# jim-berend/semanticlens

Hardware: AMD Instinct MI355X
Metric: images/sec concept-db build (higher is better)
Workload: dtype f32 (encoder GEMMs split-bf16x3, fp32 accumulate)

## Files before the change

include/semanticlens_amd.h:

```cpp
#ifndef SEMANTICLENS_AMD_H
#define SEMANTICLENS_AMD_H

#include <stddef.h>
#include <stdint.h>

#ifdef __cplusplus
extern "C" {
#endif

#define SL_ABI_VERSION 1

#define SL_E_INVALID (-1)
#define SL_E_HIP (-2)
#define SL_E_UNSUPPORTED (-3)

#define SL_F32 0
#define SL_F16 1
#define SL_BF16 2

#define SL_CONV_MAX 0
#define SL_CONV_MEAN 1
#define SL_CONV_SUM 2

#define SL_TOK_MEAN 0
// ... 126 lines not shown
                        uint16_t* d_out_split, void* stream);
int sl_attention_pool(const float* d_q, const float* d_kv, int64_t kv_row_stride, int64_t v_offset, int64_t B, int64_t T,
                      int64_t H, int64_t head_dim, float* d_out, void* stream);
int sl_patchify(const float* d_img, int64_t B, int64_t C, int64_t Hi, int64_t Wi, int64_t P, float* d_out,
                uint16_t* d_out_split, void* stream);
int sl_attention_pool_q(const float* d_q, int64_t q_batch_stride, const float* d_kv, int64_t kv_row_stride, int64_t v_offset,
                        int64_t B, int64_t T, int64_t H, int64_t head_dim, float* d_out, void* stream);
int sl_tokens_from_map(const float* d_map, int64_t B, int64_t C, int64_t S, const float* d_pos, float* d_out, void* stream);
int sl_broadcast_row(const float* d_v, const float* d_add, int64_t G, int64_t group_stride_elems, int64_t N, float* d_out,
                     void* stream);
int sl_embed_tokens(const float* d_table, int64_t vocab, const int64_t* d_ids, int64_t B, int64_t T, int64_t W,
                    const float* d_pos, float* d_out, void* stream);

#define SL_PP_SHORTEST 0
#define SL_PP_SQUASH 1
#define SL_PP_BICUBIC 0
#define SL_PP_BILINEAR 1
#define SL_PP_PLAN_STRIDE 16
#define SL_PP_INFO_WS_BYTES 0
#define SL_PP_INFO_COEF_BYTES 1
#define SL_PP_INFO_MAX_H 2
#define SL_PP_INFO_PIXEL_BYTES 3
int sl_preprocess_plan(const int32_t* h_hw, const int64_t* h_pixel_offsets, int64_t B, int S, int resize_mode,
                       int interp, int64_t* h_plan, int64_t* h_info);
int sl_preprocess(const uint8_t* d_pixels, const int64_t* d_plan, int64_t B, int S, int interp, int64_t max_h,
                  int64_t coef_bytes, const float* h_mean, const float* h_std, float* d_out, uint8_t* d_out_u8,
                  void* d_ws, size_t ws_bytes, void* stream);
int sl_preprocess_plan_rois(const int32_t* h_hw, const int64_t* h_pixel_offsets, int64_t N, const int64_t* h_index,
                            const int32_t* h_box, int64_t P, int S, int resize_mode, int interp, int64_t* h_plan,
                            int64_t* h_info);

#define SL_RENDER_CROP 0
#define SL_RENDER_OPAQUE 1
#define SL_RENDER_LIGHTEN 2
size_t sl_render_ws_bytes(int64_t B, int64_t H, int64_t W);
int sl_render_heatmaps(const float* d_rel, int64_t B, int64_t Cin, int64_t H, int64_t W, const float* d_img, int kernel_size,
                       float vis_th, float crop_th, double alpha, int style, int rf, float* d_heat, int32_t* d_box,
                       int32_t* d_flags, uint8_t* d_rgb, void* d_ws, size_t ws_bytes, void* stream);
int sl_condition_init(const float* d_act, int64_t B, int64_t C, int64_t S, int64_t sb, int64_t sc, int64_t ss,
                      const int64_t* d_channels, int rf, float* d_out, int64_t ob, int64_t oc, int64_t os, void* stream);

int sl_activation_heat_boxes(const float* d_act, int64_t B, int64_t C, int64_t S, int64_t sb, int64_t sc, int64_t ss,
                             int64_t prefix, int64_t gh, int64_t gw, const int64_t* d_rows, const int64_t* d_channels,
                             int64_t P, int64_t H, int64_t W, int kernel_size, float crop_th, float* d_heat, int32_t* d_box,
                             void* d_ws, size_t ws_bytes, void* stream);
int sl_heat_boxes(const float* d_heat, int64_t P, int64_t H, int64_t W, int kernel_size, float crop_th, int32_t* d_box,
                  void* d_ws, size_t ws_bytes, void* stream);

int sl_batchnorm_infer(const float* d_x, int64_t B, int64_t C, int64_t HW, const float* d_mean, const float* d_var,
                       const float* d_scale, const float* d_bias, double eps, int relu, float* d_y, void* stream);
int sl_batchnorm_infer_add_relu(const float* d_x, const float* d_residual, int64_t B, int64_t C, int64_t HW,
                                const float* d_mean, const float* d_var, const float* d_scale, const float* d_bias,
                                double eps, float* d_y, void* stream);

int sl_topk_init(float* d_vals, int64_t* d_ids, int64_t R, int64_t k, void* stream);
int sl_topk_merge(float* d_vals, int64_t* d_ids, int64_t R, int64_t k, const float* d_cand, int64_t ld, int64_t B,
                  int64_t id_base, void* d_ws, size_t ws_bytes, void* stream);
size_t sl_topk_merge_ws_bytes(int64_t R, int64_t k, int64_t B);
int sl_topk_merge_states(float* d_vals, int64_t* d_ids, int64_t R, int64_t k, const float* d_other_vals,
                         const int64_t* d_other_ids, int64_t M, void* stream);

int sl_cosine_nt(const float* d_x, int64_t M, const float* d_y, int64_t N, int64_t K, float* d_out, void* d_ws,
                 size_t ws_bytes, void* stream);
size_t sl_cosine_nt_ws_bytes(int64_t M, int64_t N, int64_t K);

#define SL_PROF_REDUCE 0
#define SL_PROF_MERGE 1
#define SL_PROF_GEMM 2
#define SL_PROF_GATHER 3
#define SL_PROF_SCORES 4
#define SL_PROF_BATCHNORM 5
#define SL_PROF_TOPK 6
#define SL_PROF_NFAM 7
int sl_prof_enable(int on);
int sl_prof_reset(void);
int sl_prof_read(int family, double* total_ms, int64_t* launches, double* work);

#ifdef __cplusplus
}
#endif
#endif
```

semanticlens_amd/_native.py:

```python
from __future__ import annotations

import ctypes
import operator
import os
from pathlib import Path

import torch

_PKG = Path(__file__).resolve().parent
LIB_PATH = _PKG / "lib" / "libsemanticlens_hip.so"

SL_F32, SL_F16, SL_BF16 = 0, 1, 2
SL_CONV_MAX, SL_CONV_MEAN, SL_CONV_SUM = 0, 1, 2
SL_TOK_MEAN, SL_TOK_ABSMEAN, SL_TOK_MAX, SL_TOK_ABSMAX, SL_TOK_TOKEN = 0, 1, 2, 3, 4
SL_TIES_TOTAL, SL_TIES_ATEN = 0, 1
SL_MAX_SLOTS = 16
SL_PROF_REDUCE, SL_PROF_MERGE, SL_PROF_GEMM, SL_PROF_GATHER, SL_PROF_SCORES, SL_PROF_BATCHNORM, SL_PROF_TOPK = 0, 1, 2, 3, 4, 5, 6
SL_ACT_NONE, SL_ACT_GELU, SL_ACT_QUICKGELU, SL_ACT_GELU_TANH = 0, 1, 2, 3
TIE_MODES = {"total": SL_TIES_TOTAL, "aten": SL_TIES_ATEN}
SL_PP_PLAN_STRIDE = 16
PP_RESIZE_MODES = {"shortest": 0, "squash": 1}
PP_INTERP = {"bicubic": 0, "bilinear": 1}
SL_RENDER_CROP, SL_RENDER_OPAQUE, SL_RENDER_LIGHTEN = 0, 1, 2
RENDER_STYLES = {"crop": SL_RENDER_CROP, "opaque": SL_RENDER_OPAQUE, "lighten": SL_RENDER_LIGHTEN}
# ... 28 lines not shown
    "sl_comm_destroy": (_int, [_vp]),
    "sl_comm_info": (_int, [_vp, ctypes.POINTER(_int), ctypes.POINTER(_int), ctypes.POINTER(_int)]),
    "sl_comm_allgather": (_int, [_vp, _vp, _vp, _i64, _vp]),
    "sl_comm_allreduce": (_int, [_vp, _vp, _i64, _int, _int, _vp]),
    "sl_actmax_packed_bytes": (_sz, [_int, _vp, _i64]),
    "sl_actmax_pack": (_int, [_int, _vp, _vp, _vp, _i64, _vp, _vp]),
    "sl_actmax_merge_packed": (_int, [_int, _vp, _vp, _vp, _i64, _vp, _i64, _i64, _vp]),
    "sl_actmax_allgather_merge_ws_bytes": (_sz, [_int, _vp, _i64, _int]),
    "sl_actmax_allgather_merge": (_int, [_vp, _int, _vp, _vp, _vp, _i64, _vp, _sz, _vp]),
    "sl_gather_rows": (_int, [_vp, _i64, _i64, _vp, _i64, _vp, _vp, _vp]),
    "sl_gather_rows_shard": (_int, [_vp, _i64, _i64, _vp, _i64, _i64, _i64, _vp, _vp, _vp]),
    "sl_similarity": (_int, [_vp, _i64, _i64, _vp, _i64, _i64, _vp, _vp, _sz, _vp]),
    "sl_similarity_ws_bytes": (_sz, [_i64, _i64, _i64, _i64]),
    "sl_set_gemm_mode": (_int, [_int]),
    "sl_set_reduce_policy": (_int, [_i64, _i64]),
    "sl_abs_norm_rows": (_int, [_vp, _i64, _i64, ctypes.c_float, _vp]),
    "sl_similarity_multi": (_int, [_vp, _i64, _i64, _vp, _vp, _int, _vp, _vp, _sz, _vp]),
    "sl_similarity_multi_ws_bytes": (_sz, [_i64, _i64, _vp, _int]),
    "sl_clarity": (_int, [_vp, _i64, _i64, _i64, _vp, _vp]),
    "sl_clarity_multi": (_int, [_vp, _vp, _int, _i64, _i64, _vp, _vp]),
    "sl_redundancy": (_int, [_vp, _i64, _i64, _i64, _vp, _vp, _sz, _vp]),
    "sl_redundancy_ws_bytes": (_sz, [_i64, _i64, _i64]),
    "sl_template_mean": (_int, [_vp, _vp, _i64, _i64, _i64, _vp, _vp]),
    "sl_poly2means": (_int, [_vp, _i64, _i64, _i64, _vp, _int, _vp, _int, _vp, _vp, _vp, _sz, _vp]),
    "sl_poly2means_ws_bytes": (_sz, [_i64, _i64, _i64]),
    "sl_kmeans_trials": (_int, [_int]),
    "sl_polykmeans": (_int, [_vp, _i64, _i64, _i64, _int, _vp, _int, _vp, _int, _vp, _vp, _vp, _sz, _vp]),
    "sl_polykmeans_ws_bytes": (_sz, [_i64, _i64, _i64, _int, _int]),
    "sl_linear": (_int, [_vp, _i64, _i64, _vp, _i64, _vp, _int, _vp, _vp, _i64, _i64, _i64, _i64, _vp, _vp]),
    "sl_layernorm": (_int, [_vp, _i64, _i64, _i64, _vp, _vp, ctypes.c_float, _vp, _vp, _i64, _vp]),
    "sl_attention": (_int, [_vp, _i64, _i64, _i64, _i64, _int, _vp, _vp, _vp]),
    "sl_attention_bf16x3": (_int, [_vp, _i64, _i64, _i64, _i64, _int, _vp, _vp, _vp]),
    "sl_patchify": (_int, [_vp, _i64, _i64, _i64, _i64, _i64, _vp, _vp, _vp]),
    "sl_attention_pool": (_int, [_vp, _vp, _i64, _i64, _i64, _i64, _i64, _i64, _vp, _vp]),
    "sl_attention_pool_q": (_int, [_vp, _i64, _vp, _i64, _i64, _i64, _i64, _i64, _i64, _vp, _vp]),
    "sl_tokens_from_map": (_int, [_vp, _i64, _i64, _i64, _vp, _vp, _vp]),
    "sl_split_elems": (_sz, [_i64, _i64]),
    "sl_split_bf16": (_int, [_vp, _vp, _i64, _i64, _vp, _vp]),
    "sl_linear_bf16x3": (_int, [_vp, _i64, _i64, _vp, _i64, _vp, _int, _vp, _vp, _vp, _i64, _i64, _i64, _i64, _vp, _vp]),
    "sl_broadcast_row": (_int, [_vp, _vp, _i64, _i64, _i64, _vp, _vp]),
    "sl_embed_tokens": (_int, [_vp, _i64, _vp, _i64, _i64, _i64, _vp, _vp, _vp]),
    "sl_preprocess_plan": (_int, [_vp, _vp, _i64, _int, _int, _int, _vp, _vp]),
    "sl_preprocess": (_int, [_vp, _vp, _i64, _int, _int, _i64, _i64, _vp, _vp, _vp, _vp, _vp, _sz, _vp]),
    "sl_render_ws_bytes": (_sz, [_i64, _i64, _i64]),
    "sl_render_heatmaps": (_int, [_vp, _i64, _i64, _i64, _i64, _vp, _int, ctypes.c_float, ctypes.c_float, ctypes.c_double, _int, _int,
                                  _vp, _vp, _vp, _vp, _vp, _sz, _vp]),
    "sl_condition_init": (_int, [_vp, _i64, _i64, _i64, _i64, _i64, _i64, _vp, _int, _vp, _i64, _i64, _i64, _vp]),
    "sl_preprocess_plan_rois": (_int, [_vp, _vp, _i64, _vp, _vp, _i64, _int, _int, _int, _vp, _vp]),
    "sl_activation_heat_boxes": (_int, [_vp, _i64, _i64, _i64, _i64, _i64, _i64, _i64, _i64, _i64, _vp, _vp, _i64, _i64, _i64, _int,
                                        ctypes.c_float, _vp, _vp, _vp, _sz, _vp]),
    "sl_heat_boxes": (_int, [_vp, _i64, _i64, _i64, _int, ctypes.c_float, _vp, _vp, _sz, _vp]),
    "sl_batchnorm_infer": (_int, [_vp, _i64, _i64, _i64, _vp, _vp, _vp, _vp, ctypes.c_double, _int, _vp, _vp]),
    "sl_batchnorm_infer_add_relu": (_int, [_vp, _vp, _i64, _i64, _i64, _vp, _vp, _vp, _vp, ctypes.c_double, _vp, _vp]),
    "sl_topk_init": (_int, [_vp, _vp, _i64, _i64, _vp]),
    "sl_topk_merge": (_int, [_vp, _vp, _i64, _i64, _vp, _i64, _i64, _i64, _vp, _sz, _vp]),
    "sl_topk_merge_ws_bytes": (_sz, [_i64, _i64, _i64]),
    "sl_topk_merge_states": (_int, [_vp, _vp, _i64, _i64, _vp, _vp, _i64, _vp]),
    "sl_cosine_nt": (_int, [_vp, _i64, _vp, _i64, _i64, _vp, _vp, _sz, _vp]),
    "sl_cosine_nt_ws_bytes": (_sz, [_i64, _i64, _i64]),
    "sl_prof_enable": (_int, [_int]),
    "sl_prof_reset": (_int, []),
    "sl_prof_read": (_int, [_int, ctypes.POINTER(ctypes.c_double), ctypes.POINTER(_i64), ctypes.POINTER(ctypes.c_double)]),
}

_lib = None


class NativeLibraryError(RuntimeError):
    """The HIP library is missing or a native call failed."""


def lib():
    global _lib
    if _lib is None:
        path = Path(os.environ.get("SEMANTICLENS_AMD_LIB", LIB_PATH))
        if not path.exists():
            raise NativeLibraryError(
                f"{path} not found. semanticlens_amd has no CPU fallback: build the HIP library first "
                "(python -c 'import __graft_entry__ as g; g.build()' or make -C semanticlens_amd/csrc)."
            )
        handle = ctypes.CDLL(str(path))
        for name, (res, args) in SIGNATURES.items():
            fn = getattr(handle, name)
            fn.restype = res
            fn.argtypes = args
        _lib = handle
    return _lib


def _check(rc: int, what: str) -> int:
    if rc < 0:
        msg = lib().sl_last_error().decode("utf-8", "replace")
        if rc == -1:
            raise ValueError(msg or f"{what}: invalid argument")
        raise NativeLibraryError(f"{what} failed ({rc}): {msg}")
    return rc


def default_device() -> torch.device:
    if not torch.cuda.is_available():
        raise NativeLibraryError(
            "semanticlens_amd needs a HIP device (MI355X): torch.cuda.is_available() is False and there is "
            "no CPU fallback for the concept-DB hot path."
        )
    return torch.device("cuda", torch.cuda.current_device())

# ... 623 lines not shown
    with _on(x.device):
        rc = lib().sl_cosine_nt(_ptr(x), M, _ptr(y), Nn, K, _ptr(out), _ptr(ws), ws.numel(), _stream(x))
    _check(rc, "sl_cosine_nt")
    return out


def topk_chunk_rows(R: int, n_cols: int, tile_bytes: int = TOPK_TILE_BYTES) -> int:
    return max(1, min(n_cols, tile_bytes // (4 * max(R, 1))))


def topk_probe(x: torch.Tensor, y: torch.Tensor, k: int, chunk_rows: int | None = None, id_base: int = 0, state=None):
    k = check_topk_k(k)
    if x.ndim != 2 or y.ndim != 2:
        raise ValueError("topk_probe expects 2-D tensors")
    if y.shape[1] != x.shape[1]:
        raise ValueError(f"embedding widths differ: {x.shape[1]} vs {y.shape[1]}")
    if chunk_rows is not None and chunk_rows < 1:
        raise ValueError(f"chunk_rows = {chunk_rows} must be at least 1")
    xd = _f32c(x)
    yd = _f32c(y, xd.device)
    R, n = xd.shape[0], yd.shape[0]
    vals, ids = state if state is not None else topk_new(R, k, xd.device)
    if R == 0 or n == 0:
        return vals, ids
    step = min(chunk_rows or topk_chunk_rows(R, n), n)
    tile = torch.empty(R * step, dtype=torch.float32, device=xd.device)
    ws = torch.empty(int(lib().sl_cosine_nt_ws_bytes(R, step, xd.shape[1])), dtype=torch.uint8, device=xd.device)
    merge_bytes = int(lib().sl_topk_merge_ws_bytes(R, k, step))
    merge_ws = torch.empty(merge_bytes, dtype=torch.uint8, device=xd.device) if merge_bytes else None
    for start in range(0, n, step):
        rows = min(step, n - start)
        out = tile[: R * rows].view(R, rows)
        cosine_nt(xd, yd[start : start + rows], out, ws)
        topk_merge(vals, ids, out, id_base + start, merge_ws)
    return vals, ids


BN_MAX_CHANNELS = 4096
BN_MAX_ELEMENTS = (1 << 31) - 1


def batchnorm_infer(x: torch.Tensor, mean: torch.Tensor, var: torch.Tensor, weight: torch.Tensor, bias: torch.Tensor, eps: float,
                    relu: bool = False, residual: torch.Tensor | None = None) -> torch.Tensor:
    B, C, H, W = x.shape
    out = torch.empty_like(x)
    with _on(x.device):
        if residual is None:
            rc = lib().sl_batchnorm_infer(_ptr(x), B, C, H * W, _ptr(mean), _ptr(var), _ptr(weight), _ptr(bias), float(eps),
                                          1 if relu else 0, _ptr(out), _stream(x))
        else:
            rc = lib().sl_batchnorm_infer_add_relu(_ptr(x), _ptr(residual), B, C, H * W, _ptr(mean), _ptr(var), _ptr(weight),
                                                   _ptr(bias), float(eps), _ptr(out), _stream(x))
    _check(rc, "sl_batchnorm_infer")
    return out


def prof_enable(on: bool = True):
    _check(lib().sl_prof_enable(1 if on else 0), "sl_prof_enable")


def prof_reset():
    _check(lib().sl_prof_reset(), "sl_prof_reset")


def prof_read(family: int):
    ms, n, w = ctypes.c_double(), _i64(), ctypes.c_double()
    _check(lib().sl_prof_read(family, ctypes.byref(ms), ctypes.byref(n), ctypes.byref(w)), "sl_prof_read")
    return ms.value, n.value, w.value


POLY2_MAX_N = 128


POLYK_MAX_N = 1024
POLYK_MAX_CLUSTERS = 16
POLYK_MAX_COMPONENTS = 65535


def _poly_ws_budget() -> int:
    import os

    return int(float(os.environ.get("SL_POLY_WS_GB", "8")) * (1 << 30))


def poly2means(V: torch.Tensor, first_center, rand, replace_empty_clusters: bool = True, n_clusters: int = 2) -> torch.Tensor:
    import numpy as np

    Vd = _f32c(V)
    if Vd.ndim != 3:
        raise ValueError("polysemanticity_score expects a (n_components, n_samples, n_features) tensor")
    C, n, D = Vd.shape
    first_center = np.ascontiguousarray(first_center, dtype=np.int32)
    rand = np.ascontiguousarray(rand, dtype=np.float64)
    n_init = int(first_center.shape[0])
    out = torch.empty((C,), dtype=torch.float64, device=Vd.device)
    mincnt = torch.empty((C,), dtype=torch.int32, device=Vd.device)
    general = n_clusters != 2 or n > POLY2_MAX_N
    if general:
        if n_clusters > POLYK_MAX_CLUSTERS:
            raise ValueError(f"n_clusters={n_clusters} exceeds the device kernel's maximum of {POLYK_MAX_CLUSTERS}")
        if n > POLYK_MAX_N:
            raise ValueError(f"n_samples={n} exceeds the device kernel's maximum of {POLYK_MAX_N} samples per component")
    if C == 0:
        return out
    per_comp = int(lib().sl_polykmeans_ws_bytes(1, n, D, n_clusters, n_init)) if general else int(lib().sl_poly2means_ws_bytes(1, n, D))
    chunk = max(1, min(C, POLYK_MAX_COMPONENTS, _poly_ws_budget() // max(per_comp, 1)))
# ... 385 lines not shown
```

semanticlens_amd/component_visualization/_bn_fuse.py:

```python
from __future__ import annotations

import inspect
import operator
import os
import warnings
import weakref

import torch
import torch.nn as nn
import torch.nn.functional as F

from .. import _native as N

_BN_FORWARD = nn.modules.batchnorm._BatchNorm.forward
_PLANS: "weakref.WeakKeyDictionary[nn.Module, _Plan]" = weakref.WeakKeyDictionary()
_ADDS = (operator.add, operator.iadd, torch.add)
_RELUS = (F.relu, torch.relu, torch.relu_)


def enabled() -> bool:
    return os.environ.get("SEMANTICLENS_AMD_FUSE_BN", "1") != "0"


def _plain_bn(m) -> bool:
    return isinstance(m, nn.BatchNorm2d) and type(m).forward is _BN_FORWARD


def _plain_relu(m) -> bool:
    return isinstance(m, nn.ReLU) and type(m).forward is nn.ReLU.forward


def _hooked(m: nn.Module) -> bool:
    mod = nn.modules.module
    return bool(m._forward_hooks or m._forward_pre_hooks or mod._global_forward_hooks or mod._global_forward_pre_hooks)


def _streamable(t) -> bool:
    return (isinstance(t, torch.Tensor) and t.is_cuda and t.dtype is torch.float32 and t.dim() == 4 and not t.requires_grad
            and t.is_contiguous() and not t.is_contiguous(memory_format=torch.channels_last) and t.data_ptr() % 16 == 0)


class _Site:

    __slots__ = ("bn", "verified", "dropped")

    def __init__(self, bn: nn.BatchNorm2d):
        self.bn = bn
        self.verified: set = set()
        self.dropped = False

    def eligible(self, x) -> bool:
        bn = self.bn
        if self.dropped or bn.training or torch.is_grad_enabled() or not enabled():
            return False
        if not _streamable(x) or not 0 < x.numel() <= N.BN_MAX_ELEMENTS or x.shape[1] > N.BN_MAX_CHANNELS:
            return False
        if not torch.backends.cudnn.enabled or torch.is_autocast_enabled():
            return False
        for p in (bn.running_mean, bn.running_var, bn.weight, bn.bias):
            if p is None or p.dtype is not torch.float32 or p.device != x.device or not p.is_contiguous() or p.numel() != x.shape[1]:
                return False
        return True

    def run(self, x, relu: bool, other=None, bn_first: bool = True):
        bn = self.bn
        out = N.batchnorm_infer(x, bn.running_mean, bn.running_var, bn.weight, bn.bias, bn.eps, relu=relu, residual=other)
        key = (relu, other is not None, (x.shape[2] * x.shape[3]) % 4 == 0)
        if key in self.verified:
            return out
        ref = F.batch_norm(x, bn.running_mean, bn.running_var, bn.weight, bn.bias, False, 0.0, bn.eps)
        if other is not None:
            ref = ref + other if bn_first else other + ref
        if relu:
            ref = torch.relu_(ref)
        if torch.equal(out.view(torch.int32), ref.view(torch.int32)):
            self.verified.add(key)
            return out
        self.dropped = True
        warnings.warn(
            f"the fused BatchNorm kernel did not reproduce PyTorch's result bit for bit on a {tuple(x.shape)} input "
            f"(relu={relu}, residual={other is not None}); this BatchNorm2d runs unfused from now on.", RuntimeWarning, stacklevel=3)
        return ref


def _bn_forward(site: _Site):
    def forward(x):
        if site.eligible(x):
            return site.run(x, relu=False)
        return _BN_FORWARD(site.bn, x)

    return forward


class _Fused(nn.Module):

    def __init__(self, site: _Site, relu, add=None, bn_first: bool = True):
        super().__init__()
        self.__dict__.update(site=site, relu=relu, add=add, bn_first=bn_first)

    def forward(self, x, other=None):
        site, relu = self.site, self.relu
        ok = not _hooked(site.bn) and not (isinstance(relu, nn.Module) and _hooked(relu)) and site.eligible(x)
        if ok and self.add is not None:
            ok = _streamable(other) and other.shape == x.shape and other.device == x.device
        if ok:
            return site.run(x, relu=True, other=other, bn_first=self.bn_first)
        out = site.bn(x)
        if self.add is not None:
            out = self.add(out, other) if self.bn_first else self.add(other, out)
        return relu(out)


def _trace(parent: nn.Module, sites: dict):
    from torch import fx

    class InplaceProxy(fx.Proxy):
        pass

    for name in ("iadd", "isub", "imul", "itruediv"):
        op = getattr(operator, name)
        setattr(InplaceProxy, f"__{name}__",
                lambda self, other, op=op: self.tracer.create_proxy("call_function", op, (self, other), {}))

    class LeafTracer(fx.Tracer):
        def is_leaf_module(self, m, qualname):
            return True

        def proxy(self, node):
            return InplaceProxy(node, self)

    params = list(inspect.signature(parent.forward).parameters.values())
    if any(p.kind is not p.POSITIONAL_OR_KEYWORD or p.default is not p.empty for p in params):
        return None
    graph = LeafTracer().trace(parent)
    gm = fx.GraphModule(parent, graph)
    mods = dict(parent.named_modules())

    def relu_of(node):
        if node.kwargs or len(node.args) != 1:
            return None
        if node.op == "call_module" and _plain_relu(mods.get(node.target)):
            return mods[node.target]
        if node.op == "call_function" and node.target in _RELUS:
            return F.relu
        return None

    n_fused = 0
    for node in list(graph.nodes):
        if node.op != "call_module" or mods.get(node.target) not in sites or node.kwargs or len(node.args) != 1:
            continue
        if len(node.users) != 1:
            continue
        site, user = sites[mods[node.target]], next(iter(node.users))
        last, fused, args = user, None, None
        if relu_of(user) is not None:
            fused, args = _Fused(site, relu_of(user)), (node.args[0],)
        elif (user.op == "call_function" and user.target in _ADDS and not user.kwargs and len(user.args) == 2
              and all(isinstance(a, fx.Node) for a in user.args) and user.args[0] is not user.args[1] and len(user.users) == 1):
            last = next(iter(user.users))
            if relu_of(last) is None:
                continue
            bn_first = user.args[0] is node
            if user.target is operator.iadd and not bn_first:
                continue
            fused = _Fused(site, relu_of(last), user.target, bn_first)
            args = (node.args[0], user.args[1] if bn_first else user.args[0])
        if fused is None:
            continue
        name = f"_sl_fused_{n_fused}"
        n_fused += 1
        gm.add_submodule(name, fused)
        with graph.inserting_before(last):
            new = graph.call_module(name, args)
        last.replace_all_uses_with(new)
        graph.erase_node(last)
        if last is not user:
            graph.erase_node(user)
        graph.erase_node(node)
    if not n_fused:
        return None
    graph.lint()
    gm.recompile()
    return gm


def _owner_forward(parent: nn.Module, gm, training: bool):
    own = type(parent).forward

    def forward(*args, **kwargs):
        if parent.training is training:
            return gm.forward(*args, **kwargs)
        return own(parent, *args, **kwargs)

    return forward


class _Plan:
    def __init__(self, model: nn.Module):
        self.module_ids = tuple(id(m) for m in model.modules())
        self.sites = {m: _Site(m) for m in model.modules() if _plain_bn(m) and m is not model}
        self.parents: list = []
        for parent in model.modules():
            if "forward" in parent.__dict__ or not any(child in self.sites for child in parent.children()):
                continue
            try:
                gm = _trace(parent, self.sites)
            except Exception:
                gm = None
            if gm is not None:
# ... 30 lines not shown
```

semanticlens_amd/csrc/batchnorm.hip:

```cpp
#include "common.hpp"

namespace sl {
namespace {

typedef float f4 __attribute__((ext_vector_type(4)));

enum { EPI_PLAIN = 0, EPI_RELU = 1, EPI_ADD_RELU = 2 };
enum { POL_PLAIN = 0, POL_NT_STORE = 1, POL_NT_BOTH = 2 };

constexpr int kBlock = 256;
constexpr int kUnroll = 4;
constexpr int64_t kMaxC = 4096;
constexpr int64_t kMaxTotal = (int64_t)1 << 31;

__device__ inline float bn_inv_std(float var, double eps) { return __builtin_amdgcn_rsqf(fabsf(var + (float)eps)); }

__device__ inline float bn_value(float x, const f4 k) {
  const float xhat = (x - k.x) * k.y;
  return __fmaf_rn(k.z, xhat, k.w);
}

__device__ inline float relu_clamp(float v) { return v != v ? v : fmaxf(v, 0.f); }

template <int EPI>
__device__ inline float bn_finish(float x, const f4 k, float r) {
  float y = bn_value(x, k);
  if constexpr (EPI == EPI_ADD_RELU) y = y + r;
  if constexpr (EPI != EPI_PLAIN) y = relu_clamp(y);
  return y;
}

template <int POL>
__device__ inline f4 ld4(const f4* p) {
  if constexpr (POL == POL_NT_BOTH) return __builtin_nontemporal_load(p);
  return *p;
}
template <int POL>
__device__ inline void st4(f4* p, f4 v) {
  if constexpr (POL != POL_PLAIN)
    __builtin_nontemporal_store(v, p);
  else
    *p = v;
}

template <int EPI, bool ALIGNED, int POL>
__global__ __launch_bounds__(kBlock) void batchnorm_kernel(const float* __restrict__ x, const float* __restrict__ res,
                                                           float* __restrict__ y, const float* __restrict__ mean,
                                                           const float* __restrict__ var, const float* __restrict__ scale,
                                                           const float* __restrict__ bias, double eps, uint32_t C, uint32_t HW,
                                                           uint32_t total) {
  extern __shared__ f4 tab[];
  for (uint32_t c = threadIdx.x; c < C; c += kBlock) tab[c] = f4{mean[c], bn_inv_std(var[c], eps), scale[c], bias[c]};
  __syncthreads();

  const uint32_t lane = threadIdx.x & 63;
  const uint32_t wave = blockIdx.x * (kBlock / 64) + (uint32_t)__builtin_amdgcn_readfirstlane((int)(threadIdx.x >> 6));
  const uint32_t nwaves = gridDim.x * (kBlock / 64);
  const uint32_t n4 = total / 4;
  const uint32_t per_plane = ALIGNED ? HW / 4 : 1;
  const f4* x4 = reinterpret_cast<const f4*>(x);
  const f4* r4 = reinterpret_cast<const f4*>(res);
  f4* y4 = reinterpret_cast<f4*>(y);

  for (uint32_t base = wave * (64 * kUnroll); base < n4; base += nwaves * (64 * kUnroll)) {
    f4 v[kUnroll], r[kUnroll];
#pragma unroll
    for (int u = 0; u < kUnroll; ++u) {
      const uint32_t i = base + u * 64 + lane;
      if (i < n4) {
        v[u] = ld4<POL>(x4 + i);
        if constexpr (EPI == EPI_ADD_RELU) r[u] = ld4<POL>(r4 + i);
      }
    }
#pragma unroll
    for (int u = 0; u < kUnroll; ++u) {
      const uint32_t first = base + u * 64, i = first + lane;
      if (first >= n4) break;
      f4 o;
      if constexpr (ALIGNED) {
        const uint32_t p0 = first / per_plane;
        const uint32_t last = first + 63 < n4 ? first + 63 : n4 - 1;
        uint32_t c;
        if (last - p0 * per_plane < per_plane)
          c = p0 % C;
        else
          c = (i < n4 ? i / per_plane : 0u) % C;
        if (i < n4) {
          const f4 k = tab[c];
#pragma unroll
          for (int j = 0; j < 4; ++j) o[j] = bn_finish<EPI>(v[u][j], k, EPI == EPI_ADD_RELU ? r[u][j] : 0.f);
        }
      } else {
        if (i < n4) {
          const uint32_t e = i * 4, p = e / HW;
          uint32_t off = e - p * HW, c = p % C;
#pragma unroll
          for (int j = 0; j < 4; ++j) {
            o[j] = bn_finish<EPI>(v[u][j], tab[c], EPI == EPI_ADD_RELU ? r[u][j] : 0.f);
            if (++off == HW) {
              off = 0;
              if (++c == C) c = 0;
            }
          }
        }
      }
      if (i < n4) st4<POL>(y4 + i, o);
    }
  }
  if (blockIdx.x == 0 && threadIdx.x < (total & 3u)) {
    const uint32_t e = (total & ~3u) + threadIdx.x;
    y[e] = bn_finish<EPI>(x[e], tab[(e / HW) % C], EPI == EPI_ADD_RELU ? res[e] : 0.f);
  }
}

template <int EPI, bool ALIGNED>
void launch_policy(ProfScope& prof, int pol, dim3 grid, size_t lds, hipStream_t st, const float* x, const float* res, float* y,
                   const float* mean, const float* var, const float* scale, const float* bias, double eps, uint32_t C,
                   uint32_t HW, uint32_t total) {
#define SL_BN_LAUNCH(P_) \
  SL_LAUNCH(prof, (batchnorm_kernel<EPI, ALIGNED, P_>), grid, dim3(kBlock), lds, st, x, res, y, mean, var, scale, bias, eps, C, HW, total)
  switch (pol) {
    case POL_PLAIN: SL_BN_LAUNCH(POL_PLAIN); break;
    case POL_NT_STORE: SL_BN_LAUNCH(POL_NT_STORE); break;
    default: SL_BN_LAUNCH(POL_NT_BOTH); break;
  }
#undef SL_BN_LAUNCH
}

int launch_batchnorm(int epi, const float* x, const float* res, float* y, const float* mean, const float* var,
                     const float* scale, const float* bias, double eps, int64_t B, int64_t C, int64_t HW, hipStream_t st,
                     const char* who) {
  SL_REQUIRE(B >= 0 && C >= 0 && HW >= 0, "%s: negative shape", who);
  const int64_t total = B * C * HW;
  if (total == 0) return 0;
  SL_REQUIRE(x && y && mean && var && scale && bias && (epi != EPI_ADD_RELU || res), "%s: null pointer", who);
  SL_REQUIRE(C <= kMaxC, "%s: %lld channels exceed the supported maximum of %lld", who, (long long)C, (long long)kMaxC);
  SL_REQUIRE(total < kMaxTotal, "%s: %lld elements exceed the supported maximum of 2^31 - 1", who, (long long)total);
  SL_REQUIRE((((uintptr_t)x | (uintptr_t)y | (uintptr_t)res) & 15) == 0, "%s: tensors must be 16-byte aligned", who);
  const int passes = epi == EPI_ADD_RELU ? 3 : 2;
  ProfScope prof(SL_PROF_BATCHNORM, st, (double)total * 4 * passes);
  int pol = (int)option(OPT_BN_POLICY) - 1;
  if (pol < 0 || pol > POL_NT_BOTH) pol = POL_PLAIN;
  const int64_t per_block = (int64_t)kBlock * kUnroll * 4;
  int64_t blocks = (total + per_block - 1) / per_block;
  const int64_t cap = (int64_t)num_cus() * 8;
  if (blocks > cap) blocks = cap;
  const dim3 grid((unsigned)blocks);
  const size_t lds = (size_t)C * sizeof(f4);
#define SL_BN_EPI(E_)                                                                                                      \
  if (HW % 4 == 0)                                                                                                         \
    launch_policy<E_, true>(prof, pol, grid, lds, st, x, res, y, mean, var, scale, bias, eps, (uint32_t)C, (uint32_t)HW,   \
                            (uint32_t)total);                                                                              \
  else                                                                                                                     \
    launch_policy<E_, false>(prof, pol, grid, lds, st, x, res, y, mean, var, scale, bias, eps, (uint32_t)C, (uint32_t)HW,  \
                             (uint32_t)total)
  switch (epi) {
    case EPI_PLAIN: SL_BN_EPI(EPI_PLAIN); break;
    case EPI_RELU: SL_BN_EPI(EPI_RELU); break;
    default: SL_BN_EPI(EPI_ADD_RELU); break;
  }
#undef SL_BN_EPI
  SL_CHECK_HIP(hipGetLastError());
  return 0;
}

}
}

using namespace sl;

SL_API int sl_batchnorm_infer(const float* d_x, int64_t B, int64_t C, int64_t HW, const float* d_mean, const float* d_var,
                              const float* d_scale, const float* d_bias, double eps, int relu, float* d_y, void* stream) {
  return launch_batchnorm(relu ? EPI_RELU : EPI_PLAIN, d_x, nullptr, d_y, d_mean, d_var, d_scale, d_bias, eps, B, C, HW,
                          (hipStream_t)stream, "sl_batchnorm_infer");
}

SL_API int sl_batchnorm_infer_add_relu(const float* d_x, const float* d_residual, int64_t B, int64_t C, int64_t HW,
                                       const float* d_mean, const float* d_var, const float* d_scale, const float* d_bias,
                                       double eps, float* d_y, void* stream) {
  return launch_batchnorm(EPI_ADD_RELU, d_x, d_residual, d_y, d_mean, d_var, d_scale, d_bias, eps, B, C, HW, (hipStream_t)stream,
                          "sl_batchnorm_infer_add_relu");
}
```

Measured before the change: 7289.

## Fuse BatchNorm + ReLU + max-pool into one LDS-staged kernel

Adds a fused inference kernel that applies BatchNorm and ReLU to a plane (or row band) staged in LDS, then computes the max-pool from LDS. The FX tracer now folds a following MaxPool2d / F.max_pool2d into the fused BN+ReLU site, which removes the full-resolution intermediate write and read (for example, the ResNet stem). It also makes the default BN store policy non-temporal for large tensors. The first call per shape verifies the result bit-exactly against PyTorch, and large-H planes are split into bands with halo-row re-reads.

```diff
diff --git a/include/semanticlens_amd.h b/include/semanticlens_amd.h
--- a/include/semanticlens_amd.h
+++ b/include/semanticlens_amd.h
@@ -202,6 +202,9 @@
 int sl_batchnorm_infer_add_relu(const float* d_x, const float* d_residual, int64_t B, int64_t C, int64_t HW,
                                 const float* d_mean, const float* d_var, const float* d_scale, const float* d_bias,
                                 double eps, float* d_y, void* stream);
+int sl_batchnorm_infer_relu_maxpool(const float* d_x, int64_t B, int64_t C, int64_t H, int64_t W, const float* d_mean,
+                                    const float* d_var, const float* d_scale, const float* d_bias, double eps, int kh, int kw,
+                                    int sh, int sw, int ph, int pw, float* d_y, void* stream);
 
 int sl_topk_init(float* d_vals, int64_t* d_ids, int64_t R, int64_t k, void* stream);
 int sl_topk_merge(float* d_vals, int64_t* d_ids, int64_t R, int64_t k, const float* d_cand, int64_t ld, int64_t B,
diff --git a/semanticlens_amd/_native.py b/semanticlens_amd/_native.py
--- a/semanticlens_amd/_native.py
+++ b/semanticlens_amd/_native.py
@@ -104,6 +104,8 @@
     "sl_heat_boxes": (_int, [_vp, _i64, _i64, _i64, _int, ctypes.c_float, _vp, _vp, _sz, _vp]),
     "sl_batchnorm_infer": (_int, [_vp, _i64, _i64, _i64, _vp, _vp, _vp, _vp, ctypes.c_double, _int, _vp, _vp]),
     "sl_batchnorm_infer_add_relu": (_int, [_vp, _vp, _i64, _i64, _i64, _vp, _vp, _vp, _vp, ctypes.c_double, _vp, _vp]),
+    "sl_batchnorm_infer_relu_maxpool": (_int, [_vp, _i64, _i64, _i64, _i64, _vp, _vp, _vp, _vp, ctypes.c_double, _int, _int, _int,
+                                               _int, _int, _int, _vp, _vp]),
     "sl_topk_init": (_int, [_vp, _vp, _i64, _i64, _vp]),
     "sl_topk_merge": (_int, [_vp, _vp, _i64, _i64, _vp, _i64, _i64, _i64, _vp, _sz, _vp]),
     "sl_topk_merge_ws_bytes": (_sz, [_i64, _i64, _i64]),
@@ -833,6 +835,27 @@
             rc = lib().sl_batchnorm_infer_add_relu(_ptr(x), _ptr(residual), B, C, H * W, _ptr(mean), _ptr(var), _ptr(weight),
                                                    _ptr(bias), float(eps), _ptr(out), _stream(x))
     _check(rc, "sl_batchnorm_infer")
+    return out
+
+
+BN_POOL_MAX_WIDTH = 4096
+BN_POOL_STAGE_BYTES = 64 * 1024
+
+
+def bn_pool_supported(kernel_size, stride, padding) -> bool:
+    return all(k in (2, 3) and s in (1, 2) and 0 <= p <= k // 2 for k, s, p in zip(kernel_size, stride, padding))
+
+
+def batchnorm_infer_relu_maxpool(x: torch.Tensor, mean: torch.Tensor, var: torch.Tensor, weight: torch.Tensor, bias: torch.Tensor,
+                                 eps: float, kernel_size, stride, padding) -> torch.Tensor:
+    B, C, H, W = x.shape
+    (kh, kw), (sh, sw), (ph, pw) = kernel_size, stride, padding
+    oh, ow = ((n + 2 * p - k) // s + 1 if s > 0 else 0 for n, k, s, p in ((H, kh, sh, ph), (W, kw, sw, pw)))
+    out = torch.empty((B, C, max(oh, 0), max(ow, 0)), dtype=x.dtype, device=x.device)
+    with _on(x.device):
+        rc = lib().sl_batchnorm_infer_relu_maxpool(_ptr(x), B, C, H, W, _ptr(mean), _ptr(var), _ptr(weight), _ptr(bias),
+                                                   float(eps), kh, kw, sh, sw, ph, pw, _ptr(out), _stream(x))
+    _check(rc, "sl_batchnorm_infer_relu_maxpool")
     return out
 
 
diff --git a/semanticlens_amd/component_visualization/_bn_fuse.py b/semanticlens_amd/component_visualization/_bn_fuse.py
--- a/semanticlens_amd/component_visualization/_bn_fuse.py
+++ b/semanticlens_amd/component_visualization/_bn_fuse.py
@@ -16,6 +16,7 @@
 _PLANS: "weakref.WeakKeyDictionary[nn.Module, _Plan]" = weakref.WeakKeyDictionary()
 _ADDS = (operator.add, operator.iadd, torch.add)
 _RELUS = (F.relu, torch.relu, torch.relu_)
+_POOL_ARGS = ("kernel_size", "stride", "padding", "dilation", "ceil_mode", "return_indices")
 
 
 def enabled() -> bool:
@@ -28,6 +29,28 @@
 
 def _plain_relu(m) -> bool:
     return isinstance(m, nn.ReLU) and type(m).forward is nn.ReLU.forward
+
+
+def _plain_pool(m) -> bool:
+    return isinstance(m, nn.MaxPool2d) and type(m).forward is nn.MaxPool2d.forward
+
+
+def _pair(v):
+    if isinstance(v, int) and not isinstance(v, bool):
+        return (v, v)
+    if isinstance(v, (tuple, list)) and len(v) == 2 and all(isinstance(e, int) and not isinstance(e, bool) for e in v):
+        return tuple(v)
+    return None
+
+
+def _pool_params(kernel_size, stride=None, padding=0, dilation=1, ceil_mode=False, return_indices=False):
+    if ceil_mode or return_indices or _pair(dilation) != (1, 1):
+        return None
+    k, p = _pair(kernel_size), _pair(padding)
+    s = k if stride is None or stride == [] or stride == () else _pair(stride)
+    if k is None or s is None or p is None or not N.bn_pool_supported(k, s, p):
+        return None
+    return k, s, p
 
 
 def _hooked(m: nn.Module) -> bool:
@@ -42,12 +65,13 @@
 
 class _Site:
 
-    __slots__ = ("bn", "verified", "dropped")
+    __slots__ = ("bn", "verified", "dropped", "no_pool")
 
     def __init__(self, bn: nn.BatchNorm2d):
         self.bn = bn
         self.verified: set = set()
         self.dropped = False
+        self.no_pool = False
 
     def eligible(self, x) -> bool:
         bn = self.bn
@@ -82,6 +106,31 @@
             f"(relu={relu}, residual={other is not None}); this BatchNorm2d runs unfused from now on.", RuntimeWarning, stacklevel=3)
         return ref
 
+    def pool_eligible(self, x, params) -> bool:
+        (kh, kw), _, (ph, pw) = params
+        return (not self.no_pool and x.shape[3] <= N.BN_POOL_MAX_WIDTH and x.shape[2] + 2 * ph >= kh
+                and x.shape[3] + 2 * pw >= kw)
+
+    def run_pool(self, x, params):
+        bn = self.bn
+        k, s, p = params
+        out = N.batchnorm_infer_relu_maxpool(x, bn.running_mean, bn.running_var, bn.weight, bn.bias, bn.eps, k, s, p)
+        banded = x.shape[2] > N.BN_POOL_STAGE_BYTES // (4 * x.shape[3])
+        key = ("pool", params, x.shape[3] % 4 == 0 and out.shape[3] % 4 == 0, banded)
+        if key in self.verified:
+            return out
+        ref = F.batch_norm(x, bn.running_mean, bn.running_var, bn.weight, bn.bias, False, 0.0, bn.eps)
+        ref = F.max_pool2d(torch.relu_(ref), k, s, p)
+        if out.shape == ref.shape and torch.equal(out.view(torch.int32), ref.view(torch.int32)):
+            self.verified.add(key)
+            return out
+        self.no_pool = True
+        warnings.warn(
+            f"the fused BatchNorm + ReLU + max-pool kernel did not reproduce PyTorch's result bit for bit on a {tuple(x.shape)} "
+            f"input (kernel_size={k}, stride={s}, padding={p}); this max-pool runs unfused from now on.", RuntimeWarning,
+            stacklevel=3)
+        return ref
+
 
 def _bn_forward(site: _Site):
     def forward(x):
@@ -111,6 +160,27 @@
         return relu(out)
 
 
+class _FusedPool(nn.Module):
+
+    def __init__(self, inner: _Fused, pool):
+        super().__init__()
+        self.__dict__.update(inner=inner, pool=pool)
+
+    def forward(self, x):
+        inner, pool = self.inner, self.pool
+        site, relu = inner.site, inner.relu
+        if isinstance(pool, nn.Module):
+            params = _pool_params(*(getattr(pool, name) for name in _POOL_ARGS))
+            hooked = _hooked(pool)
+        else:
+            params, hooked = _pool_params(**pool), False
+        if (params is not None and not hooked and not _hooked(site.bn) and not (isinstance(relu, nn.Module) and _hooked(relu))
+                and site.eligible(x) and site.pool_eligible(x, params)):
+            return site.run_pool(x, params)
+        out = inner(x)
+        return pool(out) if isinstance(pool, nn.Module) else F.max_pool2d(out, **pool)
+
+
 def _trace(parent: nn.Module, sites: dict):
     from torch import fx
 
@@ -143,6 +213,21 @@
             return mods[node.target]
         if node.op == "call_function" and node.target in _RELUS:
             return F.relu
+        return None
+
+    def pool_of(node, source):
+        if not node.args or node.args[0] is not source:
+            return None
+        if node.op == "call_module" and _plain_pool(mods.get(node.target)) and len(node.args) == 1 and not node.kwargs:
+            return mods[node.target]
+        if node.op == "call_function" and node.target is F.max_pool2d and len(node.args) <= 1 + len(_POOL_ARGS):
+            given = dict(zip(_POOL_ARGS, node.args[1:]))
+            if set(given) & set(node.kwargs) or not set(node.kwargs) <= set(_POOL_ARGS):
+                return None
+            given.update(node.kwargs)
+            flat = [e for v in given.values() for e in (v if isinstance(v, (tuple, list)) else (v,))]
+            if "kernel_size" in given and not any(isinstance(e, fx.Node) for e in flat):
+                return given
         return None
 
     n_fused = 0
@@ -155,6 +240,10 @@
         last, fused, args = user, None, None
         if relu_of(user) is not None:
             fused, args = _Fused(site, relu_of(user)), (node.args[0],)
+            follower = next(iter(user.users)) if len(user.users) == 1 else None
+            pool = pool_of(follower, user) if follower is not None else None
+            if pool is not None:
+                last, fused = follower, _FusedPool(fused, pool)
         elif (user.op == "call_function" and user.target in _ADDS and not user.kwargs and len(user.args) == 2
               and all(isinstance(a, fx.Node) for a in user.args) and user.args[0] is not user.args[1] and len(user.users) == 1):
             last = next(iter(user.users))
diff --git a/semanticlens_amd/csrc/batchnorm.hip b/semanticlens_amd/csrc/batchnorm.hip
--- a/semanticlens_amd/csrc/batchnorm.hip
+++ b/semanticlens_amd/csrc/batchnorm.hip
@@ -37,6 +37,18 @@
 }
 template <int POL>
 __device__ inline void st4(f4* p, f4 v) {
+  if constexpr (POL != POL_PLAIN)
+    __builtin_nontemporal_store(v, p);
+  else
+    *p = v;
+}
+template <int POL>
+__device__ inline float ld1(const float* p) {
+  if constexpr (POL == POL_NT_BOTH) return __builtin_nontemporal_load(p);
+  return *p;
+}
+template <int POL>
+__device__ inline void st1(float* p, float v) {
   if constexpr (POL != POL_PLAIN)
     __builtin_nontemporal_store(v, p);
   else
@@ -127,6 +139,14 @@
 #undef SL_BN_LAUNCH
 }
 
+constexpr int64_t kNtFromBytes = (int64_t)256 * 64 * 56 * 56 * 4;
+
+int bn_policy(int64_t tensor_bytes) {
+  const int pol = (int)option(OPT_BN_POLICY) - 1;
+  if (pol < 0 || pol > POL_NT_BOTH) return tensor_bytes >= kNtFromBytes ? POL_NT_BOTH : POL_PLAIN;
+  return pol;
+}
+
 int launch_batchnorm(int epi, const float* x, const float* res, float* y, const float* mean, const float* var,
                      const float* scale, const float* bias, double eps, int64_t B, int64_t C, int64_t HW, hipStream_t st,
                      const char* who) {
@@ -139,8 +159,7 @@
   SL_REQUIRE((((uintptr_t)x | (uintptr_t)y | (uintptr_t)res) & 15) == 0, "%s: tensors must be 16-byte aligned", who);
   const int passes = epi == EPI_ADD_RELU ? 3 : 2;
   ProfScope prof(SL_PROF_BATCHNORM, st, (double)total * 4 * passes);
-  int pol = (int)option(OPT_BN_POLICY) - 1;
-  if (pol < 0 || pol > POL_NT_BOTH) pol = POL_PLAIN;
+  const int pol = bn_policy(total * 4);
   const int64_t per_block = (int64_t)kBlock * kUnroll * 4;
   int64_t blocks = (total + per_block - 1) / per_block;
   const int64_t cap = (int64_t)num_cus() * 8;
@@ -164,6 +183,222 @@
   return 0;
 }
 
+constexpr int64_t kPoolLds = 64 * 1024;
+constexpr int64_t kLdsPerCu = 160 * 1024;
+constexpr int64_t kPoolMaxW = 4096;
+
+struct PoolGeom {
+  uint32_t C, H, W, OH, OW, kh, kw, sh, sw, ph, pw;
+  uint32_t rows, bands;
+  uint32_t nwork;
+};
+
+struct PoolBand {
+  uint32_t plane, o0, o1, r0, r1;
+  f4 k;
+};
+
+__device__ inline PoolBand pool_band(const PoolGeom& g, uint32_t work, const float* mean, const float* var, const float* scale,
+                                     const float* bias, double eps) {
+  PoolBand b;
+  b.plane = work / g.bands;
+  const uint32_t band = work - b.plane * g.bands, c = b.plane % g.C;
+  b.k = f4{mean[c], bn_inv_std(var[c], eps), scale[c], bias[c]};
+  b.o0 = band * g.rows;
+  b.o1 = b.o0 + g.rows < g.OH ? b.o0 + g.rows : g.OH;
+  const int top = (int)(b.o0 * g.sh) - (int)g.ph;
+  b.r0 = top > 0 ? (uint32_t)top : 0u;
+  const uint32_t bottom = (b.o1 - 1) * g.sh + g.kh - g.ph;
+  b.r1 = bottom < g.H ? bottom : g.H;
+  return b;
+}
+
+__device__ inline float pool_take(float m, float v) { return v > m || v != v ? v : m; }
+
+template <int KW, int SW, int PW, int POL>
+__global__ __launch_bounds__(kBlock) void bn_relu_maxpool_kernel(const float* __restrict__ x, float* __restrict__ y,
+                                                                 const float* __restrict__ mean, const float* __restrict__ var,
+                                                                 const float* __restrict__ scale, const float* __restrict__ bias,
+                                                                 double eps, const PoolGeom g) {
+  extern __shared__ f4 staged[];
+  for (uint32_t work = blockIdx.x; work < g.nwork; work += gridDim.x) {
+    const PoolBand b = pool_band(g, work, mean, var, scale, bias, eps);
+    const uint32_t w4 = g.W / 4, n4 = (b.r1 - b.r0) * w4;
+    const f4* src = reinterpret_cast<const f4*>(x + (size_t)b.plane * g.H * g.W) + (size_t)b.r0 * w4;
+    for (uint32_t base = 0; base < n4; base += kBlock * kUnroll) {
+      f4 v[kUnroll];
+#pragma unroll
+      for (int u = 0; u < kUnroll; ++u) {
+        const uint32_t i = base + u * kBlock + threadIdx.x;
+        if (i < n4) v[u] = ld4<POL>(src + i);
+      }
+#pragma unroll
+      for (int u = 0; u < kUnroll; ++u) {
+        const uint32_t i = base + u * kBlock + threadIdx.x;
+        if (i < n4) {
+          f4 o;
+#pragma unroll
+          for (int j = 0; j < 4; ++j) o[j] = relu_clamp(bn_value(v[u][j], b.k));
+          staged[i] = o;
+        }
+      }
+    }
+    __syncthreads();
+
+    constexpr int OFF = PW ? 3 : 0, SPAN = 3 * SW + KW, PIECES = (OFF + SPAN + 3) / 4;
+    constexpr float NEG_INF = -__builtin_huge_valf();
+    const uint32_t ow4 = g.OW / 4, npieces = (b.o1 - b.o0) * ow4;
+    f4* dst = reinterpret_cast<f4*>(y + (size_t)b.plane * g.OH * g.OW);
+    for (uint32_t p = threadIdx.x; p < npieces; p += kBlock) {
+      const uint32_t orow = p / ow4, q = p - orow * ow4, oh = b.o0 + orow;
+      const int col0 = (int)(q * 4 * SW) - (PW ? 4 : 0);
+      f4 m = {NEG_INF, NEG_INF, NEG_INF, NEG_INF};
+#pragma unroll
+      for (int i = 0; i < 3; ++i) {
+        const int ih = (int)(oh * g.sh) - (int)g.ph + i;
+        if (i < (int)g.kh && ih >= 0 && ih < (int)g.H) {
+          const f4* row = staged + (size_t)((uint32_t)ih - b.r0) * w4;
+          float t[PIECES * 4];
+#pragma unroll
+          for (int s = 0; s < PIECES; ++s) {
+            const int col = col0 + 4 * s;
+            const f4 piece = col >= 0 && col < (int)g.W ? row[col >> 2] : f4{NEG_INF, NEG_INF, NEG_INF, NEG_INF};
+#pragma unroll
+            for (int j = 0; j < 4; ++j) t[4 * s + j] = piece[j];
+          }
+#pragma unroll
+          for (int o = 0; o < 4; ++o) {
+#pragma unroll
+            for (int j = 0; j < KW; ++j) m[o] = pool_take(m[o], t[OFF + o * SW + j]);
+          }
+        }
+      }
+      st4<POL>(dst + (size_t)oh * ow4 + q, m);
+    }
+    __syncthreads();
+  }
+}
+
+template <int POL>
+__global__ __launch_bounds__(kBlock) void bn_relu_maxpool_scalar_kernel(const float* __restrict__ x, float* __restrict__ y,
+                                                                        const float* __restrict__ mean,
+                                                                        const float* __restrict__ var,
+                                                                        const float* __restrict__ scale,
+                                                                        const float* __restrict__ bias, double eps,
+                                                                        const PoolGeom g) {
+  extern __shared__ f4 staged[];
+  float* rows = reinterpret_cast<float*>(staged);
+  for (uint32_t work = blockIdx.x; work < g.nwork; work += gridDim.x) {
+    const PoolBand b = pool_band(g, work, mean, var, scale, bias, eps);
+    const uint32_t n = (b.r1 - b.r0) * g.W;
+    const float* src = x + (size_t)b.plane * g.H * g.W + (size_t)b.r0 * g.W;
+#pragma unroll 4
+    for (uint32_t i = threadIdx.x; i < n; i += kBlock) rows[i] = relu_clamp(bn_value(ld1<POL>(src + i), b.k));
+    __syncthreads();
+
+    const uint32_t nout = (b.o1 - b.o0) * g.OW;
+    float* dst = y + (size_t)b.plane * g.OH * g.OW;
+    for (uint32_t p = threadIdx.x; p < nout; p += kBlock) {
+      const uint32_t orow = p / g.OW, ow = p - orow * g.OW, oh = b.o0 + orow;
+      float m = -__builtin_huge_valf();
+      for (uint32_t i = 0; i < g.kh; ++i) {
+        const int ih = (int)(oh * g.sh) - (int)g.ph + (int)i;
+        if (ih < 0 || ih >= (int)g.H) continue;
+        for (uint32_t j = 0; j < g.kw; ++j) {
+          const int iw = (int)(ow * g.sw) - (int)g.pw + (int)j;
+          if (iw < 0 || iw >= (int)g.W) continue;
+          m = pool_take(m, rows[((uint32_t)ih - b.r0) * g.W + (uint32_t)iw]);
+        }
+      }
+      st1<POL>(dst + (size_t)oh * g.OW + ow, m);
+    }
+    __syncthreads();
+  }
+}
+
+template <int KW, int SW, int PW>
+void launch_pool_policy(ProfScope& prof, int pol, dim3 grid, size_t lds, hipStream_t st, const float* x, float* y,
+                        const float* mean, const float* var, const float* scale, const float* bias, double eps,
+                        const PoolGeom& g) {
+#define SL_POOL_LAUNCH(P_) \
+  SL_LAUNCH(prof, (bn_relu_maxpool_kernel<KW, SW, PW, P_>), grid, dim3(kBlock), lds, st, x, y, mean, var, scale, bias, eps, g)
+  switch (pol) {
+    case POL_PLAIN: SL_POOL_LAUNCH(POL_PLAIN); break;
+    case POL_NT_STORE: SL_POOL_LAUNCH(POL_NT_STORE); break;
+    default: SL_POOL_LAUNCH(POL_NT_BOTH); break;
+  }
+#undef SL_POOL_LAUNCH
+}
+
+int launch_bn_relu_maxpool(const float* x, float* y, const float* mean, const float* var, const float* scale, const float* bias,
+                           double eps, int64_t B, int64_t C, int64_t H, int64_t W, int kh, int kw, int sh, int sw, int ph,
+                           int pw, hipStream_t st, const char* who) {
+  SL_REQUIRE(B >= 0 && C >= 0 && H >= 0 && W >= 0, "%s: negative shape", who);
+  SL_REQUIRE((kh == 2 || kh == 3) && (kw == 2 || kw == 3), "%s: kernel size %d x %d is not supported (2 or 3 per axis)", who, kh,
+             kw);
+  SL_REQUIRE((sh == 1 || sh == 2) && (sw == 1 || sw == 2), "%s: stride %d x %d is not supported (1 or 2 per axis)", who, sh, sw);
+  SL_REQUIRE(ph >= 0 && pw >= 0 && ph <= kh / 2 && pw <= kw / 2,
+             "%s: padding %d x %d is not supported (at most half the kernel size)", who, ph, pw);
+  const int64_t total = B * C * H * W;
+  if (total == 0) return 0;
+  SL_REQUIRE(H + 2 * ph >= kh && W + 2 * pw >= kw, "%s: a %lld x %lld input is smaller than the pooling window", who,
+             (long long)H, (long long)W);
+  SL_REQUIRE(x && y && mean && var && scale && bias, "%s: null pointer", who);
+  SL_REQUIRE(C <= kMaxC, "%s: %lld channels exceed the supported maximum of %lld", who, (long long)C, (long long)kMaxC);
+  SL_REQUIRE(total < kMaxTotal, "%s: %lld elements exceed the supported maximum of 2^31 - 1", who, (long long)total);
+  SL_REQUIRE((((uintptr_t)x | (uintptr_t)y) & 15) == 0, "%s: tensors must be 16-byte aligned", who);
+  SL_REQUIRE(W <= kPoolMaxW, "%s: rows of %lld elements exceed the supported maximum of %lld", who, (long long)W,
+             (long long)kPoolMaxW);
+  PoolGeom g;
+  g.C = (uint32_t)C, g.H = (uint32_t)H, g.W = (uint32_t)W;
+  g.kh = kh, g.kw = kw, g.sh = sh, g.sw = sw, g.ph = ph, g.pw = pw;
+  g.OH = (uint32_t)((H + 2 * ph - kh) / sh + 1), g.OW = (uint32_t)((W + 2 * pw - kw) / sw + 1);
+  const int64_t fit = kPoolLds / (W * 4);
+  int64_t in_rows = H;
+  g.rows = g.OH, g.bands = 1;
+  if (H > fit) {
+    g.rows = (uint32_t)((fit - kh) / sh + 1);
+    g.bands = (g.OH + g.rows - 1) / g.rows;
+    in_rows = (int64_t)(g.rows - 1) * sh + kh;
+  }
+  const size_t lds = (size_t)(in_rows * W * 4 + 15) / 16 * 16;
+  g.nwork = (uint32_t)(B * C * g.bands);
+  int64_t per_cu = kLdsPerCu / (int64_t)lds;
+  per_cu = per_cu < 1 ? 1 : per_cu > 8 ? 8 : per_cu;
+  const int64_t cap = (int64_t)num_cus() * per_cu;
+  const dim3 grid((unsigned)(g.nwork < cap ? g.nwork : cap));
+  ProfScope prof(SL_PROF_BATCHNORM, st, ((double)total + (double)B * C * g.OH * g.OW) * 4);
+  const int pol = bn_policy(total * 4);
+  if (W % 4 == 0 && g.OW % 4 == 0) {
+#define SL_POOL_CASE(KW_, SW_, PW_)                                                                              \
+  case (KW_ - 2) * 4 + (SW_ - 1) * 2 + PW_:                                                                      \
+    launch_pool_policy<KW_, SW_, PW_>(prof, pol, grid, lds, st, x, y, mean, var, scale, bias, eps, g);           \
+    break
+    switch ((kw - 2) * 4 + (sw - 1) * 2 + pw) {
+      SL_POOL_CASE(2, 1, 0);
+      SL_POOL_CASE(2, 1, 1);
+      SL_POOL_CASE(2, 2, 0);
+      SL_POOL_CASE(2, 2, 1);
+      SL_POOL_CASE(3, 1, 0);
+      SL_POOL_CASE(3, 1, 1);
+      SL_POOL_CASE(3, 2, 0);
+      default: SL_POOL_CASE(3, 2, 1);
+    }
+#undef SL_POOL_CASE
+  } else {
+#define SL_POOL_SCALAR(P_) \
+  SL_LAUNCH(prof, (bn_relu_maxpool_scalar_kernel<P_>), grid, dim3(kBlock), lds, st, x, y, mean, var, scale, bias, eps, g)
+    switch (pol) {
+      case POL_PLAIN: SL_POOL_SCALAR(POL_PLAIN); break;
+      case POL_NT_STORE: SL_POOL_SCALAR(POL_NT_STORE); break;
+      default: SL_POOL_SCALAR(POL_NT_BOTH); break;
+    }
+#undef SL_POOL_SCALAR
+  }
+  SL_CHECK_HIP(hipGetLastError());
+  return 0;
+}
+
 }
 }
 
@@ -181,3 +416,10 @@
   return launch_batchnorm(EPI_ADD_RELU, d_x, d_residual, d_y, d_mean, d_var, d_scale, d_bias, eps, B, C, HW, (hipStream_t)stream,
                           "sl_batchnorm_infer_add_relu");
 }
+
+SL_API int sl_batchnorm_infer_relu_maxpool(const float* d_x, int64_t B, int64_t C, int64_t H, int64_t W, const float* d_mean,
+                                           const float* d_var, const float* d_scale, const float* d_bias, double eps, int kh,
+                                           int kw, int sh, int sw, int ph, int pw, float* d_y, void* stream) {
+  return launch_bn_relu_maxpool(d_x, d_y, d_mean, d_var, d_scale, d_bias, eps, B, C, H, W, kh, kw, sh, sw, ph, pw,
+                                (hipStream_t)stream, "sl_batchnorm_infer_relu_maxpool");
+}
```

After: 7502, median of 6. 2.9% higher.
